# Brown-LEMS/Edge_Based_Visual_Odometry

Measured on AMD Instinct MI355X. Metric: stereo pairs/sec (TOED+NCC match) on KITTI 1241×376; achieved HBM GB/s, higher is better.
Workload: dtype f64; 1 GPU; configs[1]: single KITTI-shaped stereo pair 1241x376 (generator S2, scene 7+rank, 12 px disparity), TOED both images (fp64, no FMA, bit-exact) + epipolar/disparity/orientation candidate search + NCC, resident in HBM, replayed; toed_mode=hybrid, edges_left=126184, edges_right=126340, candidate_pairs=581657, ncc_matches=472947, sims_stored=False, pairs_in_flight_per_gpu=6, streams_per_gpu=4, pairs_submitted_as_hipgraph=2331, toed_strict_fallbacks=0, parallelism=1 independent sequence(s), one per GPU, no collective

## Files before the change

edge_based_visual_odometry_amd/csrc/ebvo_cand.h:

```cpp
#ifndef EBVO_CAND_H
#define EBVO_CAND_H

#include "ebvo_internal.h"

#ifdef __HIPCC__
namespace
{

constexpr int CHUNK = 8;
constexpr int GROUP = 64;
constexpr double BOX_SLACK = 1e-6;

struct Box
{
    double x0, x1, y0, y1;
};

struct DevN
{
    int host;
    const int32_t *dev;
};
__device__ inline int devn(const DevN &d) { return d.dev ? *d.dev : d.host; }

struct CandParams
{
    double epi_thr, max_disp, orient_thr;
    int mask;
    DevN nL, nR;
    int64_t cap;
    int32_t *stage;
    int32_t *tile_flag;
};

__device__ inline bool box_may_match(const Box &bx, double xl, double yl, double ah, double bh, double ch,
                                     double D, double band, int mask)
{
    double x0 = bx.x0, x1 = bx.x1, y0 = bx.y0, y1 = bx.y1;
    if (mask & EBVO_STAGE_DISPARITY)
    {
        x0 = fmax(x0, xl - D);
        x1 = fmin(x1, xl + D);
        y0 = fmax(y0, yl - D);
        y1 = fmin(y1, yl + D);
        if (x0 > x1 || y0 > y1)
            return false;
    }
    if (mask & EBVO_STAGE_EPIPOLAR)
    {
        const double gx0 = ah * x0, gx1 = ah * x1, gy0 = bh * y0, gy1 = bh * y1;
        const double gmin = fmin(gx0, gx1) + fmin(gy0, gy1) + ch;
        const double gmax = fmax(gx0, gx1) + fmax(gy0, gy1) + ch;
        if (gmin > band || gmax < -band)
            return false;
    }
// ... 115 lines not shown
```

edge_based_visual_odometry_amd/csrc/ebvo_capi.hip:

```cpp
#include <chrono>
#include <cmath>
#include <cstdio>
#include <cstdlib>
#include <cstring>
#include <new>
#include <utility>

#include "ebvo_internal.h"

const char *const g_kernel_names[K_NUM] = {
    "toed_conv",   "toed_nms",   "toed_rowscan", "toed_compact", "toed_finalize", "toed_exact_centre", "toed_exact_mags", "cand_boxes", "epi_lines",
    "cand_count",  "scan",       "cand_fill",    "edge_patches", "ncc_pairs",     "ncc_stored", "misc", "sobel", "gn_refine", "sift",
    "gt_misc",     "gt_pool",    "gt_census",    "gt_rows",      "tgt_project",   "tgt_veridical", "tgt_rows",
    "pose_cascade"};

int ebvo_fail_hip(ebvo_ctx *ctx, hipError_t e, const char *what, const char *file, int line)
{
    char buf[512];
    snprintf(buf, sizeof buf, "%s failed: %s (%s:%d)", what, hipGetErrorString(e), file, line);
    if (ctx)
        ctx->last_error = buf;
    else
        fprintf(stderr, "[ebvo] %s\n", buf);
    (void)hipGetLastError();
// ... 1354 lines not shown
        return rc;
    if ((rc = ebvo_grow(ctx, s, s.keep, cp)))
        return rc;
    s.cap_pairs = cap_pairs;
    s.pipe_cap = cap_pairs;
    return EBVO_OK;
}

static int enqueue_matching(ebvo_ctx *ctx, Slot &s, int toed_mode = -1)
{
    const ebvo_stereo_params &p = s.params;
    const int h = s.cur_h, w = s.cur_w, ce = ctx->cap_edges;
    const int32_t *d_nL = s.im[0].counts + 1, *d_nR = s.im[1].counts + 1;
    int rc;
    const bool prep = !ctx->no_prep;
    const int stop = ctx->stop_stage;
    if (stop && stop <= 7)
        return EBVO_OK;
    if (prep ? (rc = match_prep_enqueue(ctx, s, h, w, ce))
             : (rc = match_lines_enqueue(ctx, s, s.d_F, s.im[0].edges, 0, d_nL, ce, (double *)s.lines.p)))
        return rc;
    if (stop == 8)
        return EBVO_OK;
    if ((rc = match_candidates_enqueue(ctx, s, s.im[0].edges, 0, d_nL, s.im[1].edges, 0, d_nR, ce,
                                       (const double *)s.lines.p, p.epi_thr, p.max_disp, p.orient_thr_deg, p.stage_mask,
                                       true, prep)))
        return rc;
    if (stop && stop <= 11)
        return EBVO_OK;
    if ((rc = match_ncc_resident_enqueue(ctx, s, h, w, ce, p.ncc_thr, 0, !(p.reserved & EBVO_PAIR_NO_SIMS), prep)))
        return rc;
    if (stop)
        return EBVO_OK;
    if ((rc = match_pair_result_enqueue(ctx, s, (toed_mode < 0 ? ctx->toed_mode : toed_mode) == EBVO_TOED_HYBRID ? ce : 0)))
        return rc;
    return EBVO_OK;
}

namespace
{
struct PackLayout
{
    size_t off[8], total;
};
__host__ __device__ inline PackLayout pack_layout(size_t nL, size_t nR, size_t np, bool theta)
{
    const size_t sizes[8] = {16 * nL, 16 * nR, theta ? 8 * nL : 0, theta ? 8 * nR : 0, 4 * (nL + 1), 4 * np, 8 * np, 8 * ((np + 63) >> 6)};
    PackLayout l;
    size_t t = 0;
    for (int k = 0; k < 8; ++k)
    {
        l.off[k] = t;
        t += (sizes[k] + 255) & ~(size_t)255;
// ... 3691 lines not shown
                               nullptr, nullptr, nullptr, (const double *)(base + o_pl), (const double *)(base + o_pr),
                               (const uint8_t *)(base + o_on), n_kf, np, tp_dist, d_rows, (uint8_t *)(base + o_tp), d_tot)))
        return rc;
    std::vector<int32_t> rows(2 * nz + 1);
    unsigned long long tot[5] = {0, 0, 0, 0, 0};
    if (n_kf)
        EBVO_HIP(ctx, hipMemcpyAsync(rows.data(), d_rows, sizeof(int32_t) * 2 * nz, hipMemcpyDeviceToHost, st));
    if (is_tp && np)
        EBVO_HIP(ctx, hipMemcpyAsync(is_tp, base + o_tp, npz, hipMemcpyDeviceToHost, st));
    EBVO_HIP(ctx, hipMemcpyAsync(tot, d_tot, sizeof tot, hipMemcpyDeviceToHost, st));
    EBVO_HIP(ctx, hipStreamSynchronize(st));
    tgt_stage_doubles(rows.data(), row_on, n_kf, stage_out);
    if ((rc = tgt_totals_agree(ctx, *stage_out, tot)))
        return rc;
    if (n_tp && n_kf)
        memcpy(n_tp, rows.data(), sizeof(int32_t) * 2 * nz);
    return EBVO_OK;
}

static bool debug_value_ok(int key, int value)
{
    switch (key)
    {
    case 4: case 7: case 10: case 13: case 14:
        return value <= 1;
    case 8:
        return value == 2 || value == 3;
    case 6:
        return value >= 1;
    case 11: case 12:
        return value <= EBVO_DEBUG_MAX_EXACT_BLOCKS;
    case 9:
        return value <= EBVO_DEBUG_MAX_GN_BLOCKS;
    case 18:
        return value <= 512;
    case 19:
        return value <= EBVO_TOTAL_PARTS;
    case 20:
        return value <= 1 << 20;
    case 21:
        return value <= EBVO_DEBUG_MAX_GT_BLOCKS;
    case 22:
        return value <= EBVO_DEBUG_MAX_TEMPORAL_BLOCKS;
    case EBVO_DEBUG_KEY_FINALIZE_BLOCKS:
        return value <= EBVO_DEBUG_MAX_FINALIZE_BLOCKS;
    case 0: case 1: case 2: case 3: case 5: case 15: case 16: case 17:
        return true;
    default:
        return false;
    }
}

extern "C" int ebvo_debug_set(ebvo_ctx *ctx, int key, int value)
{
    if (!ctx || value < 0 || !debug_value_ok(key, value))
        return EBVO_ERR_ARG;
    ++ctx->graph_gen;
    if (key == 10)
        ctx->use_graphs = value;
    else if (key == 14)
        ctx->no_prep = value;
    else if (key == 11 || key == 12)
        ctx->exact_blocks[key - 11] = value;
    else if (key == 15)
        ctx->repeat_mask = value;
    else if (key == 16)
        ctx->stop_stage = value;
    else if (key == 17)
        ctx->ncc_blocks = value;
    else if (key == 18)
        ctx->small_div = value;
    else if (key == 19)
        ctx->cand_blocks = value;
    else if (key == 20)
        ctx->pose_batch = value;
    else if (key == 21)
        ctx->gt_blocks = value;
    else if (key == 22)
        ctx->temporal_blocks = value;
    else if (key == EBVO_DEBUG_KEY_FINALIZE_BLOCKS)
        ctx->finalize_blocks = value;
    else if (key == 13)
        ctx->ingest_stream = value;
    else if (key == 0)
// ... 34 lines not shown
```

edge_based_visual_odometry_amd/csrc/ebvo_internal.h:

```cpp
#ifndef EBVO_INTERNAL_H
#define EBVO_INTERNAL_H

#include <hip/hip_runtime.h>

#include <cstddef>
#include <cstdint>
#include <string>
#include <vector>

#include "../../include/ebvo_hip.h"

enum KernelId
{
    K_CONV = 0,
    K_NMS,
    K_ROWSCAN,
    K_COMPACT,
    K_FINALIZE,
    K_EXACT_CENTRE,
    K_EXACT_MAGS,
    K_BOXES,
    K_LINES,
    K_CAND_COUNT,
    K_SCAN,
// ... 61 lines not shown

struct PairResult
{
    int32_t n_left, n_right, n_total_left, n_total_right;
    int64_t n_pairs;
    int64_t n_matches;
    int32_t overflow;
    int32_t pad;
};

struct ProfEvent
{
    hipEvent_t a, b;
    int kid;
};

constexpr int EBVO_CLEAR_MAX = 8;
constexpr int EBVO_TOTAL_PARTS = 4096;
constexpr int EBVO_MATCH_PARTS = 4096;
constexpr int EBVO_DEBUG_MAX_EXACT_BLOCKS = 65536;
constexpr int EBVO_DEBUG_MAX_GN_BLOCKS = 1 << 20;
constexpr int EBVO_DEBUG_MAX_TEMPORAL_BLOCKS = 65536;
constexpr int EBVO_DEBUG_KEY_FINALIZE_BLOCKS = 23;
constexpr int EBVO_DEBUG_MAX_FINALIZE_BLOCKS = 65536;

struct PairGraphKey
{
    int32_t h, w, toed_mode, undist;
    int64_t cap_pairs;
    uint64_t gen;
    double epi_thr, max_disp, orient_thr_deg, ncc_thr;
    int32_t stage_mask, flags;
};

struct Slot
{
    hipStream_t stream = nullptr;
    hipGraphExec_t pair_graph = nullptr;
    PairGraphKey pair_key{};
    uint64_t buf_gen = 1;
    bool pair_key_warm = false;
    bool pair_graph_off = false;
    hipStream_t own_stream = nullptr;
    hipEvent_t ev_done = nullptr;
    hipEvent_t ev_rebind = nullptr;
    struct PullMail
// ... 152 lines not shown
    std::vector<HostRange> host_ranges;
    int64_t pull_uploads = 0, stream_uploads = 0;
    hipStream_t upload_stream = nullptr;
    uint64_t sw_seq = 0;
    uint64_t sw_tag[2] = {0, 0};
    int sw_h = 0, sw_w = 0;
    PinnedBuf sw_toed[2], sw_cand, sw_ncc, sw_up;
    int gn_no_rows = 0;
    int gn_persist_waves = 2;
    int gn_persist_blocks = 0;
    int gn_per_iteration_rows = 0;
    int gn_rows_below = 0;
    int wait_attempts = 0;
    int force_overflow = 0;
    uint64_t graph_gen = 1;
    int use_graphs = 1;
    int64_t graph_launches = 0;
    int exact_blocks[2] = {0, 0};
    int cand_blocks = 0;
    int small_div = 0;
    int ncc_blocks = 0;
    int stop_stage = 0;
    int repeat_mask = 0;
    int no_prep = 0;
    int ingest_stream = 0;
    PoseRng pose_rng;
    int pose_batch = 0;
    int gt_blocks = 0;
    int temporal_blocks = 0;
    int finalize_blocks = 0;
    bool screen_audit = false;
    int64_t toed_fallbacks = 0;

    bool prof = false;
    int prof_every = 1;
    int64_t prof_submits = 0;
    std::vector<ProfEvent> prof_free;
    double prof_ms[K_NUM] = {0};
    int64_t prof_launches[K_NUM] = {0};
};

int ebvo_fail_hip(ebvo_ctx *ctx, hipError_t e, const char *what, const char *file, int line);

struct DevCount
{
    int64_t host;
// ... 42 lines not shown
    short lx, ly, rx, ry;
};
#ifdef __HIPCC__
__device__ inline bool orient_close(double a, double b, double thr)
{
    double od = fabs((a - b) * 0x1.ca5dc1a63c1f8p+5 );
    if (od > 180.0)
        od = 360.0 - od;
    return od < thr || fabs(od - 180.0) < thr;
}
#endif


int toed_init_constants(ebvo_ctx *ctx);
int toed_enqueue(ebvo_ctx *ctx, Slot &s, int n_img, int h, int w, hipEvent_t ev_conv_begin, hipEvent_t ev_conv_end,
                 hipEvent_t ev_end, int mode = -1, bool want_all4 = true);
unsigned long long *toed_screen_audit_result(Slot &s, int k, int h, int w);
void toed_screen_budget(double out[5]);

int match_lines_enqueue(ebvo_ctx *ctx, Slot &s, const double *d_F, const ebvo_edge *d_edges, int n,
                        const int32_t *d_n, int cap_n, double *d_lines);
int match_candidates_enqueue(ebvo_ctx *ctx, Slot &s, const ebvo_edge *d_L, int nL, const int32_t *d_nL,
                             const ebvo_edge *d_R, int nR, const int32_t *d_nR, int cap_edges, const double *d_lines,
                             double epi_thr, double max_disp, double orient_thr_deg, int stage_mask, bool fill, bool prep_done = false);
int match_candidates_fill_enqueue(ebvo_ctx *ctx, Slot &s, const ebvo_edge *d_L, int nL, const int32_t *d_nL,
                                  const ebvo_edge *d_R, int nR, const int32_t *d_nR, int cap_edges,
                                  const double *d_lines, double epi_thr, double max_disp, double orient_thr_deg,
                                  int stage_mask);
int match_patches_enqueue(ebvo_ctx *ctx, Slot &s, const uint8_t *d_img, int h, int w, int pitch,
                          const ebvo_edge *d_edges, int n, const int32_t *d_n, int cap_n, float *d_raw, float *d_norm,
                          uint8_t *d_flag);
int match_ncc_pairs_enqueue(ebvo_ctx *ctx, Slot &s, const uint8_t *d_imgR, int h, int w, int pitchR,
                            const ebvo_edge *d_Rc, const int32_t *d_row_ptr, int nL, int64_t n_pairs,
                            const float *d_left_norm, const uint8_t *d_left_flag, double thr, double *d_sims,
                            double *d_best, uint8_t *d_keep, int32_t *d_pair_left_scratch = nullptr,
                            void *d_sincos_scratch = nullptr ,
                            const int32_t *d_n_pairs = nullptr );
int match_ncc_resident_enqueue(ebvo_ctx *ctx, Slot &s, int h, int w, int cap_edges, double thr, int left = 0, bool want_sims = true,
                               bool prep_done = false);
int match_prep_enqueue(ebvo_ctx *ctx, Slot &s, int h, int w, int cap_edges);
size_t match_right_bank_bytes(int cap_edges);
int match_pair_result_enqueue(ebvo_ctx *ctx, Slot &s, int cand_cap);
int match_orient_flags_enqueue(ebvo_ctx *ctx, Slot &s, const ebvo_edge *d_L, int nL, const ebvo_edge *d_R, const int32_t *d_row_ptr,
                               const int32_t *d_col_idx, int64_t n_pairs, double orient_thr_deg, uint8_t *d_ok);
int match_temporal_cells_enqueue(ebvo_ctx *ctx, Slot &s, const ebvo_edge *d_cfL, const ebvo_edge *d_cfR, int n_cf, int cell, int gw,
                                 int gh, void *d_grid);
size_t match_temporal_grid_bytes(int n_cf, int n_cells);
int match_temporal_candidates_enqueue(ebvo_ctx *ctx, Slot &s, const ebvo_edge *d_kfL, const ebvo_edge *d_kfR, int n_kf,
                                      const ebvo_edge *d_cfL, const ebvo_edge *d_cfR, const void *d_grid, int n_cf, int cell,
                                      int sr, int gw, int gh, double orient_thr, int32_t *d_cnt, const int32_t *d_row_ptr,
                                      int32_t *d_col_idx, int64_t cap);
void match_temporal_grid_view(const void *d_grid, int n_cf, int n_cells, const MateCells **cells, const int32_t **cell_start,
                              const int32_t **cell_list);
int match_count_flags_enqueue(ebvo_ctx *ctx, Slot &s, const uint8_t *d_flags, int64_t n, unsigned long long *d_out,
                              const int32_t *d_n = nullptr);
int match_ncc_quads_indexed_enqueue(ebvo_ctx *ctx, Slot &s, const float *kfLn, const uint8_t *kfLf, const float *kfRn,
                                    const uint8_t *kfRf, const float *cfLn, const uint8_t *cfLf, const float *cfRn,
                                    const uint8_t *cfRf, const int32_t *d_quad_kf, const int32_t *d_quad_cf, int64_t n_quads,
                                    double thr, double *d_sim_left, double *d_sim_right, uint8_t *d_keep,
                                    const int32_t *d_n_quads = nullptr);
int ebvo_clear_enqueue(ebvo_ctx *ctx, Slot &s, int32_t *const ptrs[], const int counts[], int n);
int ebvo_device_scan(ebvo_ctx *ctx, Slot &s, const int32_t *in, int32_t *out, int n_host, const int32_t *n_dev, int n_add,
// ... 124 lines not shown
```

edge_based_visual_odometry_amd/csrc/match_kernels.hip:

```cpp
#include <atomic>
#include <cstdlib>

#include "ebvo_cand.h"
#include "ebvo_internal.h"
#include "ebvo_math.h"

namespace
{

constexpr int BATCH = 64;
constexpr int TILE = 64;
constexpr int STAGE = 64;
struct DevPairs
{
    int64_t host;
    const int32_t *row_ptr;
    DevN nL;
    int64_t cap;
};
__device__ inline int64_t devpairs(const DevPairs &d)
{
    const int64_t n = d.row_ptr ? (int64_t)d.row_ptr[devn(d.nL)] : d.host;
    return n < d.cap ? n : d.cap;
}
// ... 83 lines not shown
    const double inf = __builtin_inf();
    unsigned long long blk_total = 0;

    auto compact = [&](bool sel, int value, int *list) -> int {
        const unsigned long long m = __ballot(sel);
        if (lane == 0)
            s_wcnt[wid] = __popcll(m);
        __syncthreads();
        int pre = 0, tot = 0;
#pragma unroll
        for (int k = 0; k < 4; ++k)
        {
            if (k < wid) pre += s_wcnt[k];
            tot += s_wcnt[k];
        }
        if (sel)
            list[pre + __popcll(m & ((1ull << lane) - 1ull))] = value;
        __syncthreads();
        return tot;
    };

    if (!FILL && blockIdx.x == 0 && tid == 0)
        cnt[nL] = 0;
    if (FILL)
    {
        const int e16 = tid & 15;
        const int rows = (gridDim.x * 256) >> 4;
        for (int i = (blockIdx.x * 256 + tid) >> 4; i < nL; i += rows)
        {
            const int64_t o = row_ptr[i];
            const int n = row_ptr[i + 1] - row_ptr[i];
            if (n > STAGE)
                continue;
            for (int k = e16; k < n; k += 16)
                if (o + k < P.cap)
                    col_idx[o + k] = P.stage[(size_t)i * STAGE + k];
        }
    }
    for (int tile = blockIdx.x; tile * TILE < nL; tile += gridDim.x)
    {
        if (FILL && !P.tile_flag[tile])
            continue;
        if (wid == 0)
        {
            const int i = tile * TILE + lane;
            const bool live = i < nL;
            const int il = live ? i : 0;
// ... 818 lines not shown
        }
        const bool sent = normalise_rows(active, p, nr);
        if (active)
        {
            float4 *dst = reinterpret_cast<float4 *>(bank + (size_t)e * BANK_EDGE + side * BANK_SIDE + row * 8);
            dst[0] = make_float4(nr[0], nr[1], nr[2], nr[3]);
            dst[1] = make_float4(nr[4], nr[5], nr[6], sent ? 1.0f : 0.0f);
        }
    }
}

__device__ inline void wave_lds_sync()
{
    __builtin_amdgcn_fence(__ATOMIC_RELEASE, "workgroup");
    __builtin_amdgcn_wave_barrier();
    __builtin_amdgcn_fence(__ATOMIC_ACQUIRE, "workgroup");
}

template <int NW, int WPE>
__global__ __launch_bounds__(256, WPE) void ncc_tile_kernel(const uint8_t *__restrict__ imgL,
                                                            const uint16_t *__restrict__ pix2L, int h, int w, int pitch,
                                                       const ebvo_edge *__restrict__ L, const double2 *__restrict__ scL,
                                                       DevN nLd, const int32_t *__restrict__ row_ptr,
                                                       const int32_t *__restrict__ col_idx,
                                                       const float *__restrict__ rbank, int64_t cap, double thr,
                                                       double *__restrict__ sims, double *__restrict__ best,
                                                       uint8_t *__restrict__ keep, int32_t *__restrict__ match_part)
{
    static_assert(NW == 4, "one sampling round: four 16-lane groups, one per left edge of the tile");
    __shared__ __attribute__((aligned(16))) float s_left_all[4][NW * 2 * 7 * 8];
    __shared__ int s_mc;
    const int nL = devn(nLd);
    const int ntiles = (nL + NW - 1) / NW;
    const int per_xcd = (ntiles + 7) >> 3;
    const int xcd = blockIdx.x & 7, slot = blockIdx.x >> 3, slots = gridDim.x >> 3;
    const int t_begin = xcd * per_xcd, t_end = t_begin + per_xcd < ntiles ? t_begin + per_xcd : ntiles;
    const int wave = threadIdx.x >> 6, lane = threadIdx.x & 63;
    const int g = lane & 15, side = g >> 3, row = g & 7, r8 = lane & 7;
    float *s_left = s_left_all[wave];
    if (threadIdx.x == 0)
        s_mc = 0;
    int mc = 0;
    struct Head
    {
        int rp_l;
        double2 xy, sc;
    };
// ... 6 lines not shown
        {
            const int64_t v = row_ptr[e0 + (lane < rows ? lane : rows)];
            hd.rp_l = (int)(v < cap ? v : cap);
        }
        const int el = lane >> 4;
        const int ec = (el < rows && row < 7) ? e0 + el : 0;
        hd.xy = *reinterpret_cast<const double2 *>(&L[ec].x);
        hd.sc = scL[ec];
        return hd;
    };
    int tile = t_begin + slot * 4 + wave;
    Head cur{};
    if (tile < t_end)
        cur = load_head(tile);
    while (tile < t_end)
    {
        const int e0 = tile * NW;
        const int rows = nL - e0 < NW ? nL - e0 : NW;
        int rps[NW + 1];
#pragma unroll
        for (int t = 0; t <= NW; ++t)
            rps[t] = __builtin_amdgcn_readlane(cur.rp_l, t);
        const int k0 = rps[0], k1 = rps[NW];
        int ci_l = 0, ci_h = 0;
        if (k0 + lane < k1)
            ci_l = col_idx[k0 + lane];
        if (k0 + 64 + lane < k1)
            ci_h = col_idx[k0 + 64 + lane];
        {
            const int el = lane >> 4;
            const bool active = el < rows && row < 7;
            float p[7], nr[7];
#pragma unroll
            for (int c = 0; c < 7; ++c)
                p[c] = 0.0f;
            sample_row<true>(imgL, h, w, pitch, cur.xy.x, cur.xy.y, cur.sc.x, cur.sc.y, side, row, p, active, pix2L);
            const bool sent = normalise_rows(active, p, nr);
            if (active)
            {
                float4 *dst = reinterpret_cast<float4 *>(&s_left[((el * 2 + side) * 7 + row) * 8]);
                dst[0] = make_float4(nr[0], nr[1], nr[2], nr[3]);
                dst[1] = make_float4(nr[4], nr[5], nr[6], sent ? 1.0f : 0.0f);
            }
        }
        const int next_tile = tile + slots * 4;
        Head nxt{};
        if (next_tile < t_end)
            nxt = load_head(next_tile);
        wave_lds_sync();
        int r8l = r8;
        asm volatile("" : "+v"(r8l));
// ... 522 lines not shown
{
    if (!d_n && n <= 0)
        return EBVO_OK;
    ProfScope ps(ctx, s, K_LINES);
    hipLaunchKernelGGL(lines_kernel, dim3(blocks_for(d_n ? cap_n : n, 256, 1024)), dim3(256), 0, s.stream, d_F, d_edges,
                       DevN{n, d_n}, d_lines);
    EBVO_HIP(ctx, hipGetLastError());
    return EBVO_OK;
}

static CandParams cand_params(Slot &s, int nL, const int32_t *d_nL, int nR, const int32_t *d_nR, double epi_thr,
                              double max_disp, double orient_thr_deg, int stage_mask, int64_t cap)
{
    CandParams P;
    P.epi_thr = epi_thr;
    P.max_disp = max_disp;
    P.orient_thr = orient_thr_deg;
    P.mask = stage_mask;
    P.nL = DevN{nL, d_nL};
    P.nR = DevN{nR, d_nR};
    P.cap = cap;
    P.stage = (int32_t *)s.cand_stage.p;
    P.tile_flag = (int32_t *)s.cand_tileflag.p;
    return P;
}

int match_candidates_fill_enqueue(ebvo_ctx *ctx, Slot &s, const ebvo_edge *d_L, int nL, const int32_t *d_nL,
                                  const ebvo_edge *d_R, int nR, const int32_t *d_nR, int cap_edges,
                                  const double *d_lines, double epi_thr, double max_disp, double orient_thr_deg,
                                  int stage_mask)
{
    const CandParams P = cand_params(s, nL, d_nL, nR, d_nR, epi_thr, max_disp, orient_thr_deg, stage_mask, s.cap_pairs);
    ProfScope ps(ctx, s, K_CAND_FILL);
    hipLaunchKernelGGL(candidates_kernel<true>, dim3(blocks_for(d_nL ? cap_edges : nL, TILE, 4096 / (ctx->small_div > 0 ? ctx->small_div : 4))), dim3(256), 0,
                       s.stream, d_L, d_R, d_lines, (const Box *)s.boxes_chunk.p, (const Box *)s.boxes_group.p, P,
                       (int32_t *)nullptr, (const int32_t *)s.row_ptr.p, (int32_t *)s.col_idx.p,
                       (unsigned long long *)nullptr);
    EBVO_HIP(ctx, hipGetLastError());
    return EBVO_OK;
}

static int candidates_buffers(ebvo_ctx *ctx, Slot &s, int capL, int capR, size_t *ntiles_out, int *capgroups_out)
{
    int rc;
    if ((rc = ebvo_grow(ctx, s, s.row_ptr, sizeof(int32_t) * ((size_t)capL + 1))))
        return rc;
    if ((rc = ebvo_grow(ctx, s, s.cand_cnt, sizeof(int32_t) * ((size_t)capL + 1))))
        return rc;
    const int capchunks = (capR + CHUNK - 1) / CHUNK + 1, capgroups = (capchunks + GROUP - 1) / GROUP + 1;
    if ((rc = ebvo_grow(ctx, s, s.boxes_chunk, sizeof(Box) * (size_t)capchunks)))
        return rc;
    if ((rc = ebvo_grow(ctx, s, s.boxes_group, sizeof(Box) * (size_t)capgroups)))
        return rc;
    const size_t ntiles = ((size_t)capL + TILE - 1) / TILE + 1;
    if ((rc = ebvo_grow(ctx, s, s.cand_stage, sizeof(int32_t) * STAGE * ((size_t)capL + 1))))
// ... 24 lines not shown
    A.gb = (Box *)s.boxes_group.p;
    A.tile_flag = (int32_t *)s.cand_tileflag.p;
    A.ntiles = (int)ntiles;
    A.scL = (double2 *)s.sincos.p;
    A.scR = A.scL + cap_edges;
    A.img0 = ncc_img(s, 0);
    A.img1 = ncc_img(s, 1);
    A.pix0 = s.im[0].pix2;
    A.pix1 = s.im[1].pix2;
    A.h = h;
    A.w = w;
    A.b_lines = (int)blocks_for(cap_edges, 256, 1024);
    A.b_boxes = (int)blocks_for(capgroups, 4, 1024);
    A.b_sincos = (int)blocks_for(cap_edges, 256, 512);
    A.b_rows = (int)blocks_for(((int64_t)h * w + 3) / 4, 256, 512);
    ProfScope ps(ctx, s, K_BOXES);
    hipLaunchKernelGGL(match_prep_kernel, dim3(A.b_lines + A.b_boxes + 2 * A.b_sincos + 2 * A.b_rows), dim3(256), 0, s.stream, A);
    EBVO_HIP(ctx, hipGetLastError());
    return EBVO_OK;
}

int match_candidates_enqueue(ebvo_ctx *ctx, Slot &s, const ebvo_edge *d_L, int nL, const int32_t *d_nL,
                             const ebvo_edge *d_R, int nR, const int32_t *d_nR, int cap_edges, const double *d_lines,
                             double epi_thr, double max_disp, double orient_thr_deg, int stage_mask, bool fill, bool prep_done)
{
    const int capL = d_nL ? cap_edges : nL, capR = d_nR ? cap_edges : nR;
    int rc;
    size_t ntiles = 0;
    int capgroups = 0;
    if ((rc = candidates_buffers(ctx, s, capL, capR, &ntiles, &capgroups)))
        return rc;
    int32_t *cnt = (int32_t *)s.cand_cnt.p;
    if (!prep_done)
    {
        ProfScope ps(ctx, s, K_BOXES);
        hipLaunchKernelGGL(boxes_kernel, dim3(blocks_for(capgroups, 4, 1024)), dim3(256), 0, s.stream, d_R, DevN{nR, d_nR},
                           (Box *)s.boxes_chunk.p, (Box *)s.boxes_group.p, (int32_t *)s.cand_tileflag.p, (int)ntiles);
    }
    const CandParams P = cand_params(s, nL, d_nL, nR, d_nR, epi_thr, max_disp, orient_thr_deg, stage_mask, s.cap_pairs);
    {
        ProfScope ps(ctx, s, K_CAND_COUNT);
        const int nblk = blocks_for(capL, TILE, ctx->cand_blocks > 0 ? ctx->cand_blocks : 1024);
        s.n_total_part = nblk;
        hipLaunchKernelGGL(candidates_kernel<false>, dim3(nblk), dim3(256), 0, s.stream, d_L, d_R, d_lines,
                           (const Box *)s.boxes_chunk.p, (const Box *)s.boxes_group.p, P, cnt, (const int32_t *)nullptr,
                           (int32_t *)nullptr, s.d_total + 1);
        if (!fill)
            hipLaunchKernelGGL(total_sum_kernel, dim3(1), dim3(64), 0, s.stream,
                               (const unsigned long long *)(s.d_total + 1), nblk, s.d_total);
    }
    if (ctx->stop_stage == 9)
        return EBVO_OK;
    {
        ProfScope ps(ctx, s, K_SCAN);
        if ((rc = device_exclusive_scan(ctx, s, cnt, (int32_t *)s.row_ptr.p, DevN{nL, d_nL}, 1, capL + 1)))
            return rc;
    }
    EBVO_HIP(ctx, hipGetLastError());
    if (ctx->stop_stage == 10)
        return EBVO_OK;
    if (fill)
        return match_candidates_fill_enqueue(ctx, s, d_L, nL, d_nL, d_R, nR, d_nR, cap_edges, d_lines, epi_thr, max_disp,
                                             orient_thr_deg, stage_mask);
    return EBVO_OK;
}

int match_patches_enqueue(ebvo_ctx *ctx, Slot &s, const uint8_t *d_img, int h, int w, int pitch,
                          const ebvo_edge *d_edges, int n, const int32_t *d_n, int cap_n, float *d_raw, float *d_norm,
                          uint8_t *d_flag)
{
    if (!d_n && n <= 0)
        return EBVO_OK;
    const int cap = d_n ? cap_n : n;
    int rc;
    if ((rc = ebvo_grow(ctx, s, s.sincos, sizeof(double2) * (size_t)cap)))
        return rc;
    PatchBatch B{};
    B.img[0] = d_img;
    B.edges[0] = d_edges;
    B.n[0] = DevN{n, d_n};
    B.sc[0] = (double2 *)s.sincos.p;
    B.raw[0] = d_raw;
    B.norm[0] = d_norm;
    B.flag[0] = d_flag;
    ProfScope ps(ctx, s, K_PATCHES);
    hipLaunchKernelGGL(sincos_batch_kernel, dim3(chain_grid_cap(s, blocks_for(cap, 256, 1024)), 1), dim3(256), 0, s.stream, B);
// ... 17 lines not shown
    if (!d_sincos_scratch && (rc = ebvo_grow(ctx, s, s.sincos, sizeof(double2) * (size_t)n_pairs)))
        return rc;
    int32_t *pair_left = d_pair_left_scratch ? d_pair_left_scratch : (int32_t *)s.pair_left.p;
    double2 *sc = d_sincos_scratch ? (double2 *)d_sincos_scratch : (double2 *)s.sincos.p;
    {
        ProfScope ps(ctx, s, K_MISC);
        hipLaunchKernelGGL(expand_rows_kernel, dim3(chain_grid_cap(s, blocks_for(nL, 256, 512))), dim3(256), 0, s.stream, d_row_ptr,
                           DevN{nL, nullptr}, pair_left, n_pairs);
        hipLaunchKernelGGL(sincos_edges_kernel, dim3(chain_grid_cap(s, blocks_for(n_pairs, 256, 1024))), dim3(256), 0, s.stream, d_Rc,
                           DevN{(int)n_pairs, d_n_pairs}, sc);
    }
    {
        ProfScope ps(ctx, s, K_NCC_PAIRS);
        const int64_t threads = n_pairs * 16;
        hipLaunchKernelGGL(ncc_pairs_kernel, dim3((unsigned)((threads + 255) / 256)), dim3(256), 0, s.stream, d_imgR, h,
                           w, pitchR, d_Rc, (const double2 *)sc, (const int32_t *)pair_left, DevCount{n_pairs, d_n_pairs},
                           d_left_norm, d_left_flag, thr, d_sims, d_best, d_keep, (int32_t *)nullptr);
    }
    EBVO_HIP(ctx, hipGetLastError());
    return EBVO_OK;
}

int match_ncc_resident_enqueue(ebvo_ctx *ctx, Slot &s, int h, int w, int cap_edges, double thr, int left, bool want_sims,
                               bool prep_done)
{
    int rc;
    if ((rc = ebvo_grow(ctx, s, s.sincos, sizeof(double2) * 2 * (size_t)cap_edges)))
        return rc;
    const int iL = left ? 1 : 0, iR = 1 - iL;
    PatchBatch B{};
    for (int k = 0; k < 2; ++k)
    {
        B.img[k] = ncc_img(s, k);
        B.edges[k] = s.im[k].edges;
        B.n[k] = DevN{0, s.im[k].counts + 1};
        B.sc[k] = (double2 *)s.sincos.p + (size_t)k * cap_edges;
    }
    const DevN nLd{0, s.im[iL].counts + 1}, nRd{0, s.im[iR].counts + 1};
    {
        ProfScope ps(ctx, s, K_PATCHES);
        if (!prep_done)
        {
            hipLaunchKernelGGL(row_pairs_kernel, dim3(blocks_for(((int64_t)h * w + 3) / 4, 256, 512), 2), dim3(256), 0, s.stream,
                               ncc_img(s, 0), ncc_img(s, 1), s.im[0].pix2, s.im[1].pix2, h, w);
            hipLaunchKernelGGL(sincos_batch_kernel, dim3(blocks_for(cap_edges, 256, 512), 2), dim3(256), 0, s.stream, B);
        }
        for (int rep = 0; rep < ((ctx->repeat_mask & 4) ? 2 : 1); ++rep)
            hipLaunchKernelGGL(right_bank_kernel, dim3(blocks_for((int64_t)cap_edges * 16, 256, 1024)), dim3(256), 0, s.stream,
// ... 6 lines not shown
        ProfScope ps(ctx, s, K_NCC_PAIRS);
        int nblk = (int)blocks_for(cap_edges, NCC_NW * 4, EBVO_MATCH_PARTS);
        {
            static std::atomic<int> resident[16];
            int r = resident[ctx->device & 15].load(std::memory_order_relaxed);
            if (r == 0)
            {
                int per_cu = 0, cus = 0;
                (void)hipOccupancyMaxActiveBlocksPerMultiprocessor(&per_cu, ncc_tile_kernel<NCC_NW, NCC_WPE>, 256, 0);
                (void)hipDeviceGetAttribute(&cus, hipDeviceAttributeMultiprocessorCount, ctx->device);
                r = (per_cu > 0 ? per_cu : NCC_WPE) * (cus > 0 ? cus : 256);
                resident[ctx->device & 15].store(r, std::memory_order_relaxed);
            }
            if (ctx->ncc_blocks > 0)
                r = ctx->ncc_blocks;
            nblk = nblk < r ? nblk : r;
        }
        nblk = nblk < 8 ? 8 : (nblk & ~7);
        nblk = nblk < EBVO_MATCH_PARTS ? nblk : EBVO_MATCH_PARTS;
        s.n_match_part = nblk;
        for (int rep = 0; rep < ((ctx->repeat_mask & 8) ? 2 : 1); ++rep)
            hipLaunchKernelGGL((ncc_tile_kernel<NCC_NW, NCC_WPE>), dim3(nblk), dim3(256), 0, s.stream, ncc_img(s, iL),
                               (const uint16_t *)s.im[iL].pix2, h, w, w, (const ebvo_edge *)s.im[iL].edges,
                               (const double2 *)B.sc[iL], nLd, (const int32_t *)s.row_ptr.p, (const int32_t *)s.col_idx.p,
                               (const float *)s.patches_norm_r.p, s.cap_pairs, thr, want_sims ? (double *)s.sims.p : nullptr,
                               (double *)s.best.p, (uint8_t *)s.keep.p, s.d_matches);
    }
    EBVO_HIP(ctx, hipGetLastError());
    return EBVO_OK;
}

int match_orient_flags_enqueue(ebvo_ctx *ctx, Slot &s, const ebvo_edge *d_L, int nL, const ebvo_edge *d_R, const int32_t *d_row_ptr,
                               const int32_t *d_col_idx, int64_t n_pairs, double orient_thr_deg, uint8_t *d_ok)
{
    if (nL <= 0 || n_pairs <= 0)
        return EBVO_OK;
    ProfScope ps(ctx, s, K_CAND_FILL);
    hipLaunchKernelGGL(orient_flags_kernel, dim3(blocks_for((int64_t)nL * 16, 256, 4096)), dim3(256), 0, s.stream, d_L, nL, d_R,
                       d_row_ptr, d_col_idx, orient_thr_deg, d_ok);
    EBVO_HIP(ctx, hipGetLastError());
    return EBVO_OK;
}

size_t match_right_bank_bytes(int cap_edges) { return sizeof(float) * BANK_EDGE * (size_t)cap_edges; }


struct TemporalGrid
// ... 164 lines not shown
```

edge_based_visual_odometry_amd/csrc/toed_kernels.hip:

```cpp
#include <cstring>

#include <hip/hip_ext.h>

#include "ebvo_internal.h"
#include <atomic>
#include "ebvo_math.h"

namespace
{

const double h_TAP_INT[4][19] = {
    {7.99187055345274e-06, 6.69151128824427e-05, 0.000436341347522880, 0.00221592420596900,
     0.00876415024678427, 0.0269954832565940, 0.0647587978329459, 0.120985362259572, 0.176032663382150,
     0.199471140200716, 0.176032663382150, 0.120985362259572, 0.0647587978329459, 0.0269954832565940,
     0.00876415024678427, 0.00221592420596900, 0.000436341347522880, 6.69151128824427e-05,
     7.99187055345274e-06},
    {1.79817087452687e-05, 0.000133830225764885, 0.000763597358165040, 0.00332388630895351,
     0.0109551878084803, 0.0269954832565940, 0.0485690983747094, 0.0604926811297858, 0.0440081658455374, 0,
     -0.0440081658455374, -0.0604926811297858, -0.0485690983747094, -0.0269954832565940,
     -0.0109551878084803, -0.00332388630895351, -0.000763597358165040, -0.000133830225764885,
     -1.79817087452687e-05},
    {3.84608770384913e-05, 0.000250931673309160, 0.00122721003990810, 0.00443184841193801,
     0.0115029471989044, 0.0202466124424455, 0.0202371243227956, 0, -0.0330061243841531,
     -0.0498677850501791, -0.0330061243841531, 0, 0.0202371243227956, 0.0202466124424455,
     0.0115029471989044, 0.00443184841193801, 0.00122721003990810, 0.000250931673309160,
     3.84608770384913e-05},
    {7.75461189639711e-05, 0.000434948233735878, 0.00176581889075666, 0.00498582946343026,
     0.00890109009439027, 0.00674887081414851, -0.00910670594525801, -0.0302463405648929,
     -0.0302556140188070, 0, 0.0302556140188070, 0.0302463405648929, 0.00910670594525801,
     -0.00674887081414851, -0.00890109009439027, -0.00498582946343026, -0.00176581889075666,
     -0.000434948233735878, -7.75461189639711e-05},
};
const double h_TAP_HALF[4][19] = {
    {2.38593182706025e-05, 0.000176297841183723, 0.00101452402864988, 0.00454678125079553,
     0.0158698259178337, 0.0431386594132558, 0.0913245426945110, 0.150568716077402, 0.193334058401425,
     0.193334058401425, 0.150568716077402, 0.0913245426945110, 0.0431386594132558, 0.0158698259178337,
     0.00454678125079553, 0.00101452402864988, 0.000176297841183723, 2.38593182706025e-05,
     2.51475364429622e-06},
    {5.07010513250303e-05, 0.000330558452219480, 0.00164860154655606, 0.00625182421984385,
     0.0178535541575629, 0.0377463269865988, 0.0570778391840694, 0.0564632685290258, 0.0241667573001781,
     -0.0241667573001781, -0.0564632685290258, -0.0570778391840694, -0.0377463269865988,
     -0.0178535541575629, -0.00625182421984385, -0.00164860154655606, -0.000330558452219480,
     -5.07010513250303e-05, -5.97253990520353e-06},
    {0.000101774904498039, 0.000575722637615595, 0.00242534650599113, 0.00745956298958641,
     0.0161177919477999, 0.0222433712599600, 0.0128425138164156, -0.0164684533209659,
     -0.0453126699378339, -0.0453126699378339, -0.0164684533209659, 0.0128425138164156,
     0.0222433712599600, 0.0161177919477999, 0.00745956298958641, 0.00242534650599113,
     0.000575722637615595, 0.000101774904498039, 1.35560938637843e-05},
    {0.000190921146395817, 0.000914200719419500, 0.00311688729895755, 0.00713098700075939,
     0.00920573886249338, 0.000589786359165606, -0.0205123484567749, -0.0344073042598751,
     -0.0177474623923183, 0.0177474623923183, 0.0344073042598751, 0.0205123484567749,
     -0.000589786359165606, -0.00920573886249338, -0.00713098700075939, -0.00311688729895755,
     -0.000914200719419500, -0.000190921146395817, -2.92094529738860e-05},
};

struct ToedTables
{
    double tap_int[4][19];
    double tap_half[4][19];
    double prod_fx[17][17];
    double prod_fy[17][17];
    float screen_dc[4][2];
};
ToedTables *g_tables_dev[16] = {nullptr};

constexpr int TILE_W = 32;
constexpr int TILE_H = 8;
constexpr int HALO = 9;
constexpr int LDS_W = TILE_W + 2 * HALO;
constexpr int LDS_H = TILE_H + 2 * HALO;
constexpr int MAX_BATCH = 2;

struct CandRec
{
    double x, y, smag, tox, toy;
};

// ... 914 lines not shown
    constexpr int PM = IP ? 8 : 9;
    const bool fast = __all(window_inside(h, w, i, j));
    const ColMask cm = column_mask(w, j);
    Row24 nxt = fetch_row(img, h, w, i + PM, j);
#pragma unroll 1
    for (int p = -PM; p <= PM; ++p)
    {
        const Row24 cur = nxt;
        nxt = fetch_row(img, h, w, i - min(p + 1, PM), j);
        int vb[19];
        unpack_row(cur, h, i - p, cm, fast, vb);
        double rr[4];
#pragma unroll
        for (int d = 0; d < 4; ++d)
            rr[d] = rk[p + 9][d];
#pragma unroll
        for (int q = -PM; q <= PM; ++q)
        {
            const double v = (double)vb[q + 9];
            int lz = 0;
            if (((q + PM) & 3) == 0)
                asm volatile("" : "+v"(lz));
            const double(*ckl)[4] = ck + lz;
            double cc[4];
#pragma unroll
            for (int d = 0; d < 4; ++d)
                cc[d] = v * ckl[q + 9][d];
            if (IP)
            {
                f[0] += v * L.prod[p + 8][q + 8][0];
                f[1] += v * L.prod[p + 8][q + 8][1];
                f[2] += cc[2] * rr[0];
                f[3] += cc[1] * rr[1];
                f[4] += cc[0] * rr[2];
                f[5] += cc[2] * rr[1];
                f[6] += cc[1] * rr[2];
                f[7] += cc[3] * rr[0];
                f[8] += cc[0] * rr[3];
            }
            else
            {
                EBVO_ACCUM9(f, cc, rr)
            }
        }
    }
}

template <int SY, int SX>
__device__ inline double exact_mag(const uint8_t *__restrict__ img, int h, int w, const ExactTaps &L, int I, int J)
{
    constexpr bool IP = (SY == 0 && SX == 0);
    const int i = I >> 1, j = J >> 1;
    const double(*ck)[4] = L.tap[SX];
    const double(*rk)[4] = L.tap[SY];
    double fx = 0.0, fy = 0.0;
    constexpr int PM = IP ? 8 : 9;
    const bool fast = __all(window_inside(h, w, i, j));
    const ColMask cm = column_mask(w, j);
    Row24 nxt = fetch_row(img, h, w, i + PM, j);
#pragma unroll 1
    for (int p = -PM; p <= PM; ++p)
    {
        const Row24 cur = nxt;
        nxt = fetch_row(img, h, w, i - min(p + 1, PM), j);
        int vb[19];
        unpack_row(cur, h, i - p, cm, fast, vb);
        const double r0 = rk[p + 9][0], r1 = rk[p + 9][1];
        int lz = 0;
        asm volatile("" : "+v"(lz));
        const double(*ckl)[4] = ck + lz;
#pragma unroll
        for (int q = -PM; q <= PM; ++q)
        {
            const double v = (double)vb[q + 9];
            if (IP)
            {
                fx += v * L.prod[p + 8][q + 8][0];
                fy += v * L.prod[p + 8][q + 8][1];
            }
            else
            {
                fx += (v * ckl[q + 9][1]) * r0;
                fy += (v * ckl[q + 9][0]) * r1;
            }
        }
    }
    return sqrt(fx * fx + fy * fy);
}

#ifdef EBVO_WAVE_TRACE
__device__ unsigned long long g_wave_trace[2][8192 * 4];
__device__ inline void wave_trace(int which, int wave, unsigned long long t0, int tasks)
{
    if ((threadIdx.x & 63) == 0 && wave < 8192)
    {
        const unsigned hw = __builtin_amdgcn_s_getreg(4 | (0 << 6) | (31 << 11));
        const unsigned xcc = __builtin_amdgcn_s_getreg(20 | (0 << 6) | (31 << 11));
        unsigned long long *o = g_wave_trace[which] + (size_t)wave * 4;
        o[0] = t0;
        o[1] = __builtin_amdgcn_s_memrealtime();
        o[2] = ((unsigned long long)xcc << 32) | hw;
        o[3] = (unsigned long long)tasks;
    }
}
extern "C" int ebvo_wave_trace_read(int which, unsigned long long *dst, int n_waves)
// ... 696 lines not shown
```

Measured before the change: 3447 stereo pairs/s.

## Defer candidate row copy into NCC kernel and skip known-zero TOED taps

The candidate fill kernel no longer copies staged per-row candidate indices into col_idx. The NCC tile kernel now reads them directly from the staging buffer and writes col_idx back itself, removing a separate copy pass over the candidate list. Rows longer than the stage stride still fall back to col_idx. Separately, the exact TOED convolution loops skip multiply-adds for taps that a compile-time check proves are exactly zero, which cuts fp64 work but relies on adding +0.0 being a no-op for bit-exactness.

Result: no change. 3480 stereo pairs/s (median of 6 runs) (+1.0%).

```diff
diff --git a/edge_based_visual_odometry_amd/csrc/ebvo_cand.h b/edge_based_visual_odometry_amd/csrc/ebvo_cand.h
--- a/edge_based_visual_odometry_amd/csrc/ebvo_cand.h
+++ b/edge_based_visual_odometry_amd/csrc/ebvo_cand.h
@@ -31,6 +31,7 @@
     int64_t cap;
     int32_t *stage;
     int32_t *tile_flag;
+    int copy_rows;
 };
 
 __device__ inline bool box_may_match(const Box &bx, double xl, double yl, double ah, double bh, double ch,
diff --git a/edge_based_visual_odometry_amd/csrc/ebvo_capi.hip b/edge_based_visual_odometry_amd/csrc/ebvo_capi.hip
--- a/edge_based_visual_odometry_amd/csrc/ebvo_capi.hip
+++ b/edge_based_visual_odometry_amd/csrc/ebvo_capi.hip
@@ -1400,13 +1400,14 @@
         return rc;
     if (stop == 8)
         return EBVO_OK;
+    const bool staged = !ctx->no_staged_rows && !(stop && stop <= 12);
     if ((rc = match_candidates_enqueue(ctx, s, s.im[0].edges, 0, d_nL, s.im[1].edges, 0, d_nR, ce,
                                        (const double *)s.lines.p, p.epi_thr, p.max_disp, p.orient_thr_deg, p.stage_mask,
-                                       true, prep)))
+                                       true, prep, !staged)))
         return rc;
     if (stop && stop <= 11)
         return EBVO_OK;
-    if ((rc = match_ncc_resident_enqueue(ctx, s, h, w, ce, p.ncc_thr, 0, !(p.reserved & EBVO_PAIR_NO_SIMS), prep)))
+    if ((rc = match_ncc_resident_enqueue(ctx, s, h, w, ce, p.ncc_thr, 0, !(p.reserved & EBVO_PAIR_NO_SIMS), prep, staged)))
         return rc;
     if (stop)
         return EBVO_OK;
@@ -5144,7 +5145,7 @@
 {
     switch (key)
     {
-    case 4: case 7: case 10: case 13: case 14:
+    case 4: case 7: case 10: case 13: case 14: case EBVO_DEBUG_KEY_NO_STAGED_ROWS:
         return value <= 1;
     case 8:
         return value == 2 || value == 3;
@@ -5182,6 +5183,8 @@
         ctx->use_graphs = value;
     else if (key == 14)
         ctx->no_prep = value;
+    else if (key == EBVO_DEBUG_KEY_NO_STAGED_ROWS)
+        ctx->no_staged_rows = value;
     else if (key == 11 || key == 12)
         ctx->exact_blocks[key - 11] = value;
     else if (key == 15)
diff --git a/edge_based_visual_odometry_amd/csrc/ebvo_internal.h b/edge_based_visual_odometry_amd/csrc/ebvo_internal.h
--- a/edge_based_visual_odometry_amd/csrc/ebvo_internal.h
+++ b/edge_based_visual_odometry_amd/csrc/ebvo_internal.h
@@ -107,6 +107,7 @@
 constexpr int EBVO_DEBUG_MAX_GN_BLOCKS = 1 << 20;
 constexpr int EBVO_DEBUG_MAX_TEMPORAL_BLOCKS = 65536;
 constexpr int EBVO_DEBUG_KEY_FINALIZE_BLOCKS = 23;
+constexpr int EBVO_DEBUG_KEY_NO_STAGED_ROWS = 25;
 constexpr int EBVO_DEBUG_MAX_FINALIZE_BLOCKS = 65536;
 
 struct PairGraphKey
@@ -305,6 +306,7 @@
     int ncc_blocks = 0;
     int stop_stage = 0;
     int repeat_mask = 0;
+    int no_staged_rows = 0;
     int no_prep = 0;
     int ingest_stream = 0;
     PoseRng pose_rng;
@@ -393,11 +395,12 @@
                         const int32_t *d_n, int cap_n, double *d_lines);
 int match_candidates_enqueue(ebvo_ctx *ctx, Slot &s, const ebvo_edge *d_L, int nL, const int32_t *d_nL,
                              const ebvo_edge *d_R, int nR, const int32_t *d_nR, int cap_edges, const double *d_lines,
-                             double epi_thr, double max_disp, double orient_thr_deg, int stage_mask, bool fill, bool prep_done = false);
+                             double epi_thr, double max_disp, double orient_thr_deg, int stage_mask, bool fill, bool prep_done = false,
+                             bool copy_rows = true );
 int match_candidates_fill_enqueue(ebvo_ctx *ctx, Slot &s, const ebvo_edge *d_L, int nL, const int32_t *d_nL,
                                   const ebvo_edge *d_R, int nR, const int32_t *d_nR, int cap_edges,
                                   const double *d_lines, double epi_thr, double max_disp, double orient_thr_deg,
-                                  int stage_mask);
+                                  int stage_mask, bool copy_rows = true);
 int match_patches_enqueue(ebvo_ctx *ctx, Slot &s, const uint8_t *d_img, int h, int w, int pitch,
                           const ebvo_edge *d_edges, int n, const int32_t *d_n, int cap_n, float *d_raw, float *d_norm,
                           uint8_t *d_flag);
@@ -408,7 +411,7 @@
                             void *d_sincos_scratch = nullptr ,
                             const int32_t *d_n_pairs = nullptr );
 int match_ncc_resident_enqueue(ebvo_ctx *ctx, Slot &s, int h, int w, int cap_edges, double thr, int left = 0, bool want_sims = true,
-                               bool prep_done = false);
+                               bool prep_done = false, bool staged_rows = false);
 int match_prep_enqueue(ebvo_ctx *ctx, Slot &s, int h, int w, int cap_edges);
 size_t match_right_bank_bytes(int cap_edges);
 int match_pair_result_enqueue(ebvo_ctx *ctx, Slot &s, int cand_cap);
diff --git a/edge_based_visual_odometry_amd/csrc/match_kernels.hip b/edge_based_visual_odometry_amd/csrc/match_kernels.hip
--- a/edge_based_visual_odometry_amd/csrc/match_kernels.hip
+++ b/edge_based_visual_odometry_amd/csrc/match_kernels.hip
@@ -129,7 +129,7 @@
 
     if (!FILL && blockIdx.x == 0 && tid == 0)
         cnt[nL] = 0;
-    if (FILL)
+    if (FILL && P.copy_rows)
     {
         const int e16 = tid & 15;
         const int rows = (gridDim.x * 256) >> 4;
@@ -994,7 +994,7 @@
                                                             const uint16_t *__restrict__ pix2L, int h, int w, int pitch,
                                                        const ebvo_edge *__restrict__ L, const double2 *__restrict__ scL,
                                                        DevN nLd, const int32_t *__restrict__ row_ptr,
-                                                       const int32_t *__restrict__ col_idx,
+                                                       int32_t *col_idx, const int32_t *__restrict__ stage, int stage_stride,
                                                        const float *__restrict__ rbank, int64_t cap, double thr,
                                                        double *__restrict__ sims, double *__restrict__ best,
                                                        uint8_t *__restrict__ keep, int32_t *__restrict__ match_part)
@@ -1047,11 +1047,39 @@
         for (int t = 0; t <= NW; ++t)
             rps[t] = __builtin_amdgcn_readlane(cur.rp_l, t);
         const int k0 = rps[0], k1 = rps[NW];
+        auto staged_index = [&](int k) {
+            int el = 0, s0 = rps[0], s1 = rps[1];
+#pragma unroll
+            for (int t = 1; t < NW; ++t)
+                if (t < rows && k >= rps[t])
+                {
+                    el = t;
+                    s0 = rps[t];
+                    s1 = rps[t + 1];
+                }
+            if (s1 - s0 > stage_stride)
+                return col_idx[k];
+            const int v = stage[(size_t)(e0 + el) * stage_stride + (k - s0)];
+            col_idx[k] = v;
+            return v;
+        };
         int ci_l = 0, ci_h = 0;
-        if (k0 + lane < k1)
-            ci_l = col_idx[k0 + lane];
-        if (k0 + 64 + lane < k1)
-            ci_h = col_idx[k0 + 64 + lane];
+        if (stage)
+        {
+            if (k0 + lane < k1)
+                ci_l = staged_index(k0 + lane);
+            if (k0 + 64 + lane < k1)
+                ci_h = staged_index(k0 + 64 + lane);
+            for (int k = k0 + 128 + lane; k < k1; k += 64)
+                (void)staged_index(k);
+        }
+        else
+        {
+            if (k0 + lane < k1)
+                ci_l = col_idx[k0 + lane];
+            if (k0 + 64 + lane < k1)
+                ci_h = col_idx[k0 + 64 + lane];
+        }
         {
             const int el = lane >> 4;
             const bool active = el < rows && row < 7;
@@ -1620,15 +1648,17 @@
     P.cap = cap;
     P.stage = (int32_t *)s.cand_stage.p;
     P.tile_flag = (int32_t *)s.cand_tileflag.p;
+    P.copy_rows = 1;
     return P;
 }
 
 int match_candidates_fill_enqueue(ebvo_ctx *ctx, Slot &s, const ebvo_edge *d_L, int nL, const int32_t *d_nL,
                                   const ebvo_edge *d_R, int nR, const int32_t *d_nR, int cap_edges,
                                   const double *d_lines, double epi_thr, double max_disp, double orient_thr_deg,
-                                  int stage_mask)
-{
-    const CandParams P = cand_params(s, nL, d_nL, nR, d_nR, epi_thr, max_disp, orient_thr_deg, stage_mask, s.cap_pairs);
+                                  int stage_mask, bool copy_rows)
+{
+    CandParams P = cand_params(s, nL, d_nL, nR, d_nR, epi_thr, max_disp, orient_thr_deg, stage_mask, s.cap_pairs);
+    P.copy_rows = copy_rows ? 1 : 0;
     ProfScope ps(ctx, s, K_CAND_FILL);
     hipLaunchKernelGGL(candidates_kernel<true>, dim3(blocks_for(d_nL ? cap_edges : nL, TILE, 4096 / (ctx->small_div > 0 ? ctx->small_div : 4))), dim3(256), 0,
                        s.stream, d_L, d_R, d_lines, (const Box *)s.boxes_chunk.p, (const Box *)s.boxes_group.p, P,
@@ -1699,7 +1729,8 @@
 
 int match_candidates_enqueue(ebvo_ctx *ctx, Slot &s, const ebvo_edge *d_L, int nL, const int32_t *d_nL,
                              const ebvo_edge *d_R, int nR, const int32_t *d_nR, int cap_edges, const double *d_lines,
-                             double epi_thr, double max_disp, double orient_thr_deg, int stage_mask, bool fill, bool prep_done)
+                             double epi_thr, double max_disp, double orient_thr_deg, int stage_mask, bool fill, bool prep_done,
+                             bool copy_rows)
 {
     const int capL = d_nL ? cap_edges : nL, capR = d_nR ? cap_edges : nR;
     int rc;
@@ -1738,7 +1769,7 @@
         return EBVO_OK;
     if (fill)
         return match_candidates_fill_enqueue(ctx, s, d_L, nL, d_nL, d_R, nR, d_nR, cap_edges, d_lines, epi_thr, max_disp,
-                                             orient_thr_deg, stage_mask);
+                                             orient_thr_deg, stage_mask, copy_rows);
     return EBVO_OK;
 }
 
@@ -1802,8 +1833,10 @@
 }
 
 int match_ncc_resident_enqueue(ebvo_ctx *ctx, Slot &s, int h, int w, int cap_edges, double thr, int left, bool want_sims,
-                               bool prep_done)
-{
+                               bool prep_done, bool staged_rows)
+{
+    if (staged_rows && (left || !s.cand_stage.p))
+        return EBVO_ERR_ARG;
     int rc;
     if ((rc = ebvo_grow(ctx, s, s.sincos, sizeof(double2) * 2 * (size_t)cap_edges)))
         return rc;
@@ -1856,7 +1889,8 @@
         for (int rep = 0; rep < ((ctx->repeat_mask & 8) ? 2 : 1); ++rep)
             hipLaunchKernelGGL((ncc_tile_kernel<NCC_NW, NCC_WPE>), dim3(nblk), dim3(256), 0, s.stream, ncc_img(s, iL),
                                (const uint16_t *)s.im[iL].pix2, h, w, w, (const ebvo_edge *)s.im[iL].edges,
-                               (const double2 *)B.sc[iL], nLd, (const int32_t *)s.row_ptr.p, (const int32_t *)s.col_idx.p,
+                               (const double2 *)B.sc[iL], nLd, (const int32_t *)s.row_ptr.p, (int32_t *)s.col_idx.p,
+                               staged_rows ? (const int32_t *)s.cand_stage.p : (const int32_t *)nullptr, STAGE,
                                (const float *)s.patches_norm_r.p, s.cap_pairs, thr, want_sims ? (double *)s.sims.p : nullptr,
                                (double *)s.best.p, (uint8_t *)s.keep.p, s.d_matches);
     }
diff --git a/edge_based_visual_odometry_amd/csrc/toed_kernels.hip b/edge_based_visual_odometry_amd/csrc/toed_kernels.hip
--- a/edge_based_visual_odometry_amd/csrc/toed_kernels.hip
+++ b/edge_based_visual_odometry_amd/csrc/toed_kernels.hip
@@ -9,7 +9,7 @@
 namespace
 {
 
-const double h_TAP_INT[4][19] = {
+constexpr double h_TAP_INT[4][19] = {
     {7.99187055345274e-06, 6.69151128824427e-05, 0.000436341347522880, 0.00221592420596900,
      0.00876415024678427, 0.0269954832565940, 0.0647587978329459, 0.120985362259572, 0.176032663382150,
      0.199471140200716, 0.176032663382150, 0.120985362259572, 0.0647587978329459, 0.0269954832565940,
@@ -31,7 +31,7 @@
      -0.00674887081414851, -0.00890109009439027, -0.00498582946343026, -0.00176581889075666,
      -0.000434948233735878, -7.75461189639711e-05},
 };
-const double h_TAP_HALF[4][19] = {
+constexpr double h_TAP_HALF[4][19] = {
     {2.38593182706025e-05, 0.000176297841183723, 0.00101452402864988, 0.00454678125079553,
      0.0158698259178337, 0.0431386594132558, 0.0913245426945110, 0.150568716077402, 0.193334058401425,
      0.193334058401425, 0.150568716077402, 0.0913245426945110, 0.0431386594132558, 0.0158698259178337,
@@ -53,6 +53,21 @@
      -0.000589786359165606, -0.00920573886249338, -0.00713098700075939, -0.00311688729895755,
      -0.000914200719419500, -0.000190921146395817, -2.92094529738860e-05},
 };
+
+constexpr bool tap_is_zero(bool half, int d, int k)
+{
+    return !half && ((d == 1 && k == 9) || (d == 2 && (k == 7 || k == 11)) || (d == 3 && k == 9));
+}
+constexpr bool taps_match_zero_predicate()
+{
+    for (int d = 0; d < 4; ++d)
+        for (int k = 0; k < 19; ++k)
+            if ((h_TAP_INT[d][k] == 0.0) != tap_is_zero(false, d, k) || (h_TAP_HALF[d][k] == 0.0) != tap_is_zero(true, d, k))
+                return false;
+    return true;
+}
+static_assert(taps_match_zero_predicate(), "tap_is_zero must name exactly the zero taps of h_TAP_INT / h_TAP_HALF");
+static_assert(h_TAP_INT[1][9] == 0.0 && h_TAP_INT[0][9] > 0.0, "prod_fx[p][8] and prod_fy[8][q] are +0.0");
 
 struct ToedTables
 {
@@ -1013,26 +1028,26 @@
             if (((q + PM) & 3) == 0)
                 asm volatile("" : "+v"(lz));
             const double(*ckl)[4] = ck + lz;
+            const bool z1 = tap_is_zero(SX, 1, q + 9), z2 = tap_is_zero(SX, 2, q + 9), z3 = tap_is_zero(SX, 3, q + 9);
             double cc[4];
 #pragma unroll
             for (int d = 0; d < 4; ++d)
-                cc[d] = v * ckl[q + 9][d];
-            if (IP)
-            {
-                f[0] += v * L.prod[p + 8][q + 8][0];
-                f[1] += v * L.prod[p + 8][q + 8][1];
+                cc[d] = tap_is_zero(SX, d, q + 9) ? 0.0 : v * ckl[q + 9][d];
+            if (!z1)
+                f[0] += IP ? v * L.prod[p + 8][q + 8][0] : cc[1] * rr[0];
+            f[1] += IP ? v * L.prod[p + 8][q + 8][1] : cc[0] * rr[1];
+            if (!z2)
                 f[2] += cc[2] * rr[0];
+            if (!z1)
                 f[3] += cc[1] * rr[1];
-                f[4] += cc[0] * rr[2];
+            f[4] += cc[0] * rr[2];
+            if (!z2)
                 f[5] += cc[2] * rr[1];
+            if (!z1)
                 f[6] += cc[1] * rr[2];
+            if (!z3)
                 f[7] += cc[3] * rr[0];
-                f[8] += cc[0] * rr[3];
-            }
-            else
-            {
-                EBVO_ACCUM9(f, cc, rr)
-            }
+            f[8] += cc[0] * rr[3];
         }
     }
 }
@@ -1064,14 +1079,17 @@
         for (int q = -PM; q <= PM; ++q)
         {
             const double v = (double)vb[q + 9];
+            const bool z1 = tap_is_zero(SX, 1, q + 9);
             if (IP)
             {
-                fx += v * L.prod[p + 8][q + 8][0];
+                if (!z1)
+                    fx += v * L.prod[p + 8][q + 8][0];
                 fy += v * L.prod[p + 8][q + 8][1];
             }
             else
             {
-                fx += (v * ckl[q + 9][1]) * r0;
+                if (!z1)
+                    fx += (v * ckl[q + 9][1]) * r0;
                 fy += (v * ckl[q + 9][0]) * r1;
             }
         }
```
